# burlachenkok/flpytorch

Measured on AMD Instinct MI355X. Metric: gradient-codec encode+reduce GB/s (device-resident), [N,D] fp32; % HBM peak, higher is better.
Workload: dtype f32; 1 GPU; C3 topk:1% N=1024/GPU D=10000000; codec=topk:1%, clients_per_gpu=1024, clients_total=1024, D=10000000, K=100000, rows_alloc=contiguous, parallelism=client-shard dp1

## Files before the change

flpytorch_amd/csrc/select.hip:

```cpp
#include <stdlib.h>

#include <atomic>
#include <map>
#include <mutex>
#include <vector>

#include "chunks.hpp"
#include "randk_tree.hpp"

namespace flc {

constexpr uint32_t ALL = 0xFFFFFFFFu;
constexpr uint32_t F_OVERFLOW = 1u, F_SHORT = 2u, F_TIES = 4u, F_EXACT = 8u;
constexpr uint32_t F_RESIDENT = 16u;
constexpr uint32_t F_REPAIR = 32u;
constexpr int SMAX = 16384;
constexpr int HBINS = 2048;
constexpr uint32_t TIECAP = HBINS;
constexpr int CS_SH = 64;
constexpr int64_t CS_FEW = 16;
constexpr int CS_ST = 8;
constexpr int CS_LCAP = 2048;
constexpr int RS_U = 16;
#ifndef FLC_RS_NG
// ... 73 lines not shown
    uint32_t* krem;
    uint32_t* tieprefix;
    uint32_t* tiecut;
    uint32_t* hist;
    uint32_t* worklist;
    uint32_t* nwork;
    uint32_t* cursor;
    uint32_t* cstate;
    uint64_t* clist;
    uint32_t* carrive;
    uint32_t* shcnt;
    uint32_t* zm;
    float* part;
    int64_t cap;
    uint32_t tie_hi;
};

__device__ __host__ inline uint32_t tie_pref(uint32_t ix, uint32_t hi) { return hi ? ix : ~ix; }
__device__ __host__ inline uint32_t tie_all(uint32_t hi) { return hi ? 0u : 0xFFFFFFFFu; }


__device__ inline void lds_bar() {
    asm volatile("s_waitcnt lgkmcnt(0)" ::: "memory");
    __builtin_amdgcn_s_barrier();
    asm volatile("" ::: "memory");
}
template <bool RAW>
__device__ inline void blk_bar() {
    if (RAW) lds_bar();
    else __syncthreads();
}
// ... 201 lines not shown
        for (int i = threadIdx.x; i < HBINS; i += NT) ws.hist[row * HBINS + i] = 0;
}

#ifndef FLC_CS_NT
#define FLC_CS_NT 1
#endif
__device__ inline float4 cs_ld(const float4* p) {
#if FLC_CS_NT
    typedef float v4f __attribute__((ext_vector_type(4)));
    const v4f v = __builtin_nontemporal_load(reinterpret_cast<const v4f*>(p));
    return make_float4(v.x, v.y, v.z, v.w);
#else
    return *p;
#endif
}
template <int NT>
__device__ void cand_select_row(int64_t row, int64_t K, SelWs ws, uint32_t* h, uint32_t* scratch) {
    {
        if (ws.flags[row]) return;
        const uint32_t cnt = ws.rowcnt[(row) * RCS];
        if (cnt < (uint32_t)K) {
            if (threadIdx.x == 0) ws.flags[row] |= F_SHORT;
            return;
        }
        const uint32_t T = ws.thr[row];
        const uint32_t span = ws.prefix[row] - T;
        int s = 0;
        while (s < 21 && (((uint64_t)span * 4u) >> s) >= (uint64_t)HBINS) ++s;
        const float* vals = ws.ent_val + row * ws.cap;
        const float4* v4 = reinterpret_cast<const float4*>(vals);
        const uint32_t n4 = cnt >> 2;
        uint32_t prefix = 0, krem = (uint32_t)K, last = 0;
// ... 36 lines not shown
        }
        __syncthreads();
        const uint32_t thr = T + prefix;
        bool ties = !fail && last > krem;
        if (ties && last > TIECAP) { fail = true; ties = false; }
        if (ties) {
            uint32_t* tix = h;
            if (threadIdx.x == 0) scratch[0] = 0;
            __syncthreads();
            const uint32_t* idxs = ws.ent_idx + row * ws.cap;
            for (uint32_t i = threadIdx.x; i < n4; i += NT) {
                const float4 q = v4[i];
                const float qv[4] = {q.x, q.y, q.z, q.w};
#pragma unroll
                for (int u = 0; u < 4; ++u)
                    if (mag_key(qv[u]) == thr) tix[atomicAdd(&scratch[0], 1u)] = idxs[i * 4 + u];
            }
            for (uint32_t i = n4 * 4 + threadIdx.x; i < cnt; i += NT) {
                if (mag_key(vals[i]) == thr) tix[atomicAdd(&scratch[0], 1u)] = idxs[i];
            }
            __syncthreads();
            const uint32_t m = scratch[0];
            for (uint32_t a = threadIdx.x; a < m; a += NT) {
                const uint32_t ia = tix[a];
                uint32_t rank = 0;
                for (uint32_t b = 0; b < m; ++b) rank += tie_pref(tix[b], ws.tie_hi) > tie_pref(ia, ws.tie_hi) ? 1u : 0u;
                if (rank == krem - 1) ws.tiecut[row] = ia;
            }
        }
        if (threadIdx.x == 0) {
            if (fail) {
                ws.flags[row] |= F_SHORT;
            } else {
                ws.thr[row] = thr;
                ws.krem[row] = krem;
                if (ties) ws.flags[row] |= F_TIES;
            }
// ... 351 lines not shown
#define FLC_TK_STPOL 0
#endif
#ifndef FLC_TK_COPY4
#define FLC_TK_COPY4 1
#endif
#ifndef FLC_TK_PROBE
#define FLC_TK_PROBE 0
#endif

template <int POL = FLC_TK_STPOL>
__device__ inline void tk_copy_out(const uint32_t* si, const uint32_t* sv, const SelWs& ws, int64_t n, int64_t row,
                                   uint32_t pos, uint32_t tot, bool fits, int lane, int64_t wslot) {
    int64_t at = row * ws.cap + pos;
    if (FLC_TK_PROBE == 4) at = (wslot % max((n * ws.cap) >> 10, (int64_t)1)) << 10;
    const uint32_t nrec = (fits && FLC_TK_PROBE != 2) ? tot * 4u : 0u;
    const auto di = __builtin_amdgcn_make_buffer_rsrc(ws.ent_idx + at, (short)0, (int)nrec, 0x00020000);
    const auto dv = __builtin_amdgcn_make_buffer_rsrc(ws.ent_val + at, (short)0, (int)nrec, 0x00020000);
    typedef unsigned int u4v __attribute__((ext_vector_type(4)));
    const uint32_t nq = min(tot, (uint32_t)GCAP) >> 2;
#pragma unroll
    for (int k = 0; k < GCAP / 256; ++k) {
        const uint32_t q = (uint32_t)(k * 64 + lane);
        const uint4 a = reinterpret_cast<const uint4*>(si)[q];
        const uint4 b = reinterpret_cast<const uint4*>(sv)[q];
        const uint32_t off = q < nq ? q * 16u : 0x7FFFFFF0u;
        __builtin_amdgcn_raw_buffer_store_b128(__builtin_bit_cast(u4v, a), di, off, 0, POL);
        __builtin_amdgcn_raw_buffer_store_b128(__builtin_bit_cast(u4v, b), dv, off, 0, POL);
    }
    const uint32_t e = nq * 4u + (uint32_t)(lane & 3);
    const uint32_t off = lane < 3 ? e * 4u : 0x7FFFFFF0u;
    __builtin_amdgcn_raw_buffer_store_b32(si[e], di, off, 0, POL);
    __builtin_amdgcn_raw_buffer_store_b32(sv[e], dv, off, 0, POL);
}

template <int RING, int FGS, int LONE = 0>
#ifndef FLC_TK_RING
#define FLC_TK_RING 16
#endif
#ifndef FLC_TK_WPE
#define FLC_TK_WPE 1
#endif
__global__ __launch_bounds__(256) __attribute__((amdgpu_waves_per_eu(FLC_TK_WPE))) void k_topk_filter_fast(RowSrc rows, int64_t n, int64_t r0, int64_t rn, int64_t rb, int64_t d, SelWs ws, int shards,
                                                                                                float* __restrict__ zout) {
    static_assert(16 % RING == 0, "ring must divide the 16 loads of a chunk");
    constexpr int SROW = GCAP + 64;
    static_assert((SROW * 4) % 256 == 0, "value block offset in 256-byte units");
    __shared__ __attribute__((aligned(16))) uint32_t st[2][4][2 * SROW];
// ... 144 lines not shown
#endif
#ifndef FLC_TK_WG_STPOL
#define FLC_TK_WG_STPOL 17
#endif
#ifndef FLC_TK_WG_WPE
#define FLC_TK_WG_WPE 4
#endif
__device__ inline uint32_t lds_addr(const void* p) {
    return (uint32_t)(size_t)(const __attribute__((address_space(3))) void*)p;
}
__device__ inline uint32_t lds_peek(uint32_t addr) {
    uint32_t v;
    asm volatile("ds_read_b32 %0, %1\n\ts_waitcnt lgkmcnt(0)" : "=&v"(v) : "v"(addr) : "memory");
    return __builtin_amdgcn_readfirstlane(v);
}
template <int RING, int NL>
__global__ __launch_bounds__((NL + 1) * 64) __attribute__((amdgpu_waves_per_eu(FLC_TK_WG_WPE))) void k_topk_filter_fast_wg(RowSrc rows, int64_t n, int64_t r0, int64_t rn, int64_t rb, int64_t d,
                                                                        SelWs ws) {
    static_assert(16 % RING == 0, "ring must divide the 16 loads of a chunk");
    constexpr int FGS = 4;
    constexpr int SROW = GCAP + 64;
    __shared__ __attribute__((aligned(16))) uint32_t st[2][NL][2 * SROW];
    __shared__ __attribute__((aligned(16))) uint32_t hs[2][NL][4];
    __shared__ uint32_t fr[2];
    const int lane = threadIdx.x & 63;
    const int wv = __builtin_amdgcn_readfirstlane(threadIdx.x >> 6);
    if (threadIdx.x < 2 * NL * 4) (&hs[0][0][0])[threadIdx.x] = 0;
    if (threadIdx.x < 2) fr[threadIdx.x] = 0;
    __syncthreads();
    const int64_t C = nchunks(d);
    const int64_t G = (C + FGS * NL - 1) / (FGS * NL);
// ... 47 lines not shown
                for (int w = 0; w < NL; ++w)
                    if ((lane >> 2) == w) {
                        off = pre[w];
                        gf = tot[w] <= GCAP;
#pragma unroll
                        for (int u = 0; u < FGS; ++u) {
                            const uint32_t x = (uint32_t)(cc[w] >> (16 * u)) & 0xFFFFu;
                            off += u < (lane & 3) ? x : 0u;
                            cu = u == (lane & 3) ? x : cu;
                        }
                    }
                ws.tab[(c0 + lane) * n + row] = make_uint2(base + off, fits && gf ? cu : 0u);
            }
            if (!(fits && allfit) && lane == 0) atomicOr(&ws.flags[row], F_OVERFLOW);
#pragma unroll
            for (int w = 0; w < NL; ++w)
                tk_copy_out<FLC_TK_WG_STPOL>(st[b][w], st[b][w] + SROW, ws, n, row, base + pre[w], tot[w], fits && tot[w] <= GCAP, lane,
                            (int64_t)blockIdx.x * NL + w);
            asm volatile("s_waitcnt lgkmcnt(0)\n\tds_write_b32 %0, %1" ::"v"(lds_addr(&fr[b])), "v"(k + 1) : "memory");
        }
        return;
    }
    float4 ring[RING];
    int64_t row, c;
    item_at(it, row, c);
    c += wv * FGS;
    auto rs = chunk_rsrc(rows.row_s(row), c * CHUNK, d);
#pragma unroll
    for (int L = 0; L < RING - 1; ++L) {
        ring[L] = load_q(rs, lane, L);
        __builtin_amdgcn_sched_barrier(0);
    }
    for (uint32_t k = 0; it < items; ++k) {
// ... 156 lines not shown
    }
    if (lane == 63) wsum[wv] = inc;
    __syncthreads();
    uint32_t before = 0, tot = 0;
#pragma unroll
    for (int k = 0; k < NT / 64; ++k) {
        const uint32_t x = wsum[k];
        before += k < wv ? x : 0u;
        tot += x;
    }
    __syncthreads();
    total = tot;
    return before + inc - v;
}

template <bool VEC, int NT = EX_NT>
__device__ void exact_row(RowSrc rows, int64_t n, int64_t row, int64_t d, int64_t K, SelWs ws, uint32_t* h,
                          uint32_t* scratch, uint32_t* wsum) {
    const int t = threadIdx.x;
    const int64_t C = nchunks(d);
    {
        const float* r = rows.row(row);
        uint32_t prefix = 0, krem = (uint32_t)K, ties_tot = 0;
        for (int p = 0; p < 3; ++p) {
            for (int i = t; i < HBINS; i += NT) h[i] = 0;
            __syncthreads();
            auto add = [&](uint32_t k) { if (key_in_prefix(k, p, prefix)) atomicAdd(&h[key_bin(k, p)], 1u); };
            int64_t j = 0;
            if (VEC) {
                const float4* r4 = reinterpret_cast<const float4*>(r);
                const int64_t g4 = d / 4;
// ... 54 lines not shown
            }
            uint32_t etot;
            uint32_t erank = tie_run + ex_scan<NT>(ne, wsum, etot);
            uint32_t na = 0;
            bool adm[4];
#pragma unroll
            for (int q = 0; q < 4; ++q) {
                adm[q] = gt[q] || (eq[q] && erank >= tie_from && erank < tie_to);
                erank += eq[q] ? 1u : 0u;
                na += adm[q] ? 1u : 0u;
            }
            uint32_t atot;
            uint32_t pos = base + ex_scan<NT>(na, wsum, atot);
#pragma unroll
            for (int q = 0; q < 4; ++q)
                if (adm[q]) { oi[pos] = (uint32_t)(j0 + q); ov[pos] = v[q]; ++pos; }
            base += atot;
            tie_run += etot;
            if (sb == SUBS - 1 && t == 0) ws.tab[c * n + row] = make_uint2(cbase, base - cbase);
        }
        if (t == 0) {
            ws.thr[row] = thr;
            ws.krem[row] = krem;
            ws.rowcnt[row * RCS] = base;
            ws.flags[row] = F_EXACT | (ws.flags[row] & (F_OVERFLOW | F_SHORT));
        }
        __syncthreads();
    }
}

template <bool VEC>
__global__ __launch_bounds__(EX_NT) void k_topk_exact_rows(RowSrc rows, int64_t n, int64_t r0, int64_t rn, int64_t d, int64_t K, SelWs ws) {
    __shared__ uint32_t h[HBINS];
    __shared__ uint32_t scratch[260];
    __shared__ uint32_t wsum[EX_NT / 64];
    for (int64_t row = r0 + blockIdx.x; row < r0 + rn; row += gridDim.x) {
        if (!(ws.flags[row] & (F_OVERFLOW | F_SHORT))) continue;
        exact_row<VEC>(rows, n, row, d, K, ws, h, scratch, wsum);
    }
}

template <int NT, bool VEC>
__global__ __launch_bounds__(NT) void k_cand_select_x(RowSrc rows, int64_t n, int64_t r0, int64_t rn, int64_t d, int64_t K,
                                                      SelWs ws) {
    __shared__ uint32_t h[HBINS];
    __shared__ uint32_t scratch[260];
    __shared__ uint32_t wsum[NT / 64];
    __shared__ uint32_t failed;
    for (int64_t row = r0 + blockIdx.x; row < r0 + rn; row += gridDim.x) {
        cand_select_row<NT>(row, K, ws, h, scratch);
        __syncthreads();
        if (threadIdx.x == 0) failed = __atomic_load_n(&ws.flags[row], __ATOMIC_RELAXED) & (F_OVERFLOW | F_SHORT);
        __syncthreads();
        if (failed) exact_row<VEC, NT>(rows, n, row, d, K, ws, h, scratch, wsum);
        __syncthreads();
    }
}

__global__ __launch_bounds__(256) void k_tie_count(RowSrc rows, int64_t n, int64_t d, SelWs ws) {
    const int64_t C = nchunks(d);
    const int lane = threadIdx.x & 63, wv = threadIdx.x >> 6;
    const int64_t nrows = *ws.nwork;
    const int64_t bpr = (C + 3) / 4;
    for (int64_t it = blockIdx.x; it < nrows * bpr; it += gridDim.x) {
        const int64_t row = ws.worklist[it / bpr];
        const int64_t c = (it % bpr) * 4 + wv;
        if (c >= C) continue;
        uint32_t cnt = 0;
        if (ws.flags[row] & F_TIES) {
// ... 264 lines not shown
    m.te = make_uint2(0, 0);
    m.thr = 0; m.cut = 0u; m.mode = 0; m.w = 1.f;
    if (r < (rend < 0 ? n : rend)) {
        m.te = ws.tab[c * n + r];
        m.thr = ws.thr[r];
        const uint32_t f = ws.flags[r];
        m.mode = (f & F_EXACT) ? 2u : ((f & F_TIES) ? 1u : 0u);
        if (m.mode == 1u) m.cut = tie_pref(ws.tiecut[r], ws.tie_hi);
        if (m.mode == 2u) m.thr = 0u;
        if (w) m.w = w[r];
    }
    return m;
}


template <int TS>
__device__ void resolve_neg_zero(float* tl, uint32_t* rm, const SelWs& ws, int64_t c, int64_t n, uint32_t cbase,
                                 int64_t len, const float* w, int lane) {
    constexpr int NW = TS / 32;
    constexpr int WL = (NW + 63) / 64;
    bool any = false;
    for (int k = 0; k < TS / 64; ++k) {
        const int64_t i = (int64_t)k * 64 + lane;
        const uint64_t b = __ballot(i < len && __float_as_uint(tl[i]) == 0x80000000u);
        if (lane == 0) { rm[2 * k] = (uint32_t)b; rm[2 * k + 1] = (uint32_t)(b >> 32); }
        any |= b != 0ull;
    }
    if (!any) return;
    uint32_t z0[WL], zc[WL];
#pragma unroll
    for (int j = 0; j < WL; ++j) {
        const int k = lane + 64 * j;
        z0[j] = k < NW ? rm[k] : 0u;
        zc[j] = z0[j];
    }
    for (int64_t r = 0; r < n; ++r) {
        if (w && (__float_as_uint(w[r]) >> 31)) continue;
#pragma unroll
        for (int j = 0; j < WL; ++j) if (lane + 64 * j < NW) rm[lane + 64 * j] = 0u;
        const RowMeta m = load_meta(ws, c, n, r, w);
        const uint32_t mode = m.mode, T = m.thr, cut = m.cut;
        for (uint32_t e = (uint32_t)lane; e < m.te.y; e += 64) {
            const uint32_t ix = ws.ent_idx[r * ws.cap + m.te.x + e];
            const uint32_t key = mag_key(ws.ent_val[r * ws.cap + m.te.x + e]);
            const uint32_t loc = ix - cbase;
            if (loc < (uint32_t)TS && (mode == 2u || key > T || (key == T && tie_pref(ix, ws.tie_hi) >= cut)))
                atomicOr(&rm[loc >> 5], 1u << (loc & 31));
        }
        bool left = false;
#pragma unroll
        for (int j = 0; j < WL; ++j) {
            if (lane + 64 * j < NW) zc[j] &= rm[lane + 64 * j];
            left |= zc[j] != 0u;
        }
        if (__ballot(left) == 0ull) break;
    }
#pragma unroll
    for (int j = 0; j < WL; ++j) {
        uint32_t dead = z0[j] & ~zc[j];
        while (dead) {
            const int b = __builtin_ctz(dead);
            dead &= dead - 1u;
            tl[(lane + 64 * j) * 32 + b] = 0.f;
        }
    }
}

template <int TS>
__device__ void resolve_neg_zero_g(float* tl, uint32_t* rm, const SelWs& ws, int64_t c, int64_t n, uint32_t cbase,
                                   int64_t len, const float* w, int lane) {
    constexpr int NW = TS / 32;
    constexpr int WL = (NW + 63) / 64;
    uint32_t z0[WL], zc[WL];
#pragma unroll
    for (int j = 0; j < WL; ++j) z0[j] = 0u;
    bool any = false;
#pragma unroll 4
    for (int k = 0; k < TS / 64; ++k) {
        const int64_t i = (int64_t)k * 64 + lane;
        const uint64_t b = __ballot(i < len && __float_as_uint(tl[i]) == 0x80000000u);
        const int w0 = 2 * k, w1 = 2 * k + 1;
#pragma unroll
        for (int j = 0; j < WL; ++j) {
// ... 1 lines not shown
            if (lane == (w1 & 63) && (w1 >> 6) == j) z0[j] = (uint32_t)(b >> 32);
        }
        any |= b != 0ull;
    }
    if (!any) return;
#pragma unroll
    for (int j = 0; j < WL; ++j) zc[j] = z0[j];
    for (int64_t r = 0; r < n; ++r) {
        if (w && (__float_as_uint(w[r]) >> 31)) continue;
#pragma unroll
        for (int j = 0; j < WL; ++j) if (lane + 64 * j < NW) rm[lane + 64 * j] = 0u;
        __threadfence_block();
        const RowMeta m = load_meta(ws, c, n, r, w);
        const uint32_t mode = m.mode, T = m.thr, cut = m.cut;
        for (uint32_t e = (uint32_t)lane; e < m.te.y; e += 64) {
            const uint32_t ix = ws.ent_idx[r * ws.cap + m.te.x + e];
            const uint32_t key = mag_key(ws.ent_val[r * ws.cap + m.te.x + e]);
            const uint32_t loc = ix - cbase;
            if (loc < (uint32_t)TS && (mode == 2u || key > T || (key == T && tie_pref(ix, ws.tie_hi) >= cut)))
                atomicOr(&rm[loc >> 5], 1u << (loc & 31));
        }
        __threadfence_block();
        bool left = false;
#pragma unroll
        for (int j = 0; j < WL; ++j) {
            if (lane + 64 * j < NW) zc[j] &= atomicOr(&rm[lane + 64 * j], 0u);
            left |= zc[j] != 0u;
        }
        if (__ballot(left) == 0ull) break;
    }
#pragma unroll
    for (int j = 0; j < WL; ++j) {
        uint32_t dead = z0[j] & ~zc[j];
        while (dead) {
            const int b = __builtin_ctz(dead);
            dead &= dead - 1u;
            tl[(lane + 64 * j) * 32 + b] = 0.f;
        }
    }
}

template <bool ASSIGN, int TS, bool W, int WPB, int AP = AP>
__device__ __forceinline__ void chunk_accum_body(int64_t n, int64_t d, SelWs ws, const float* __restrict__ w, float wt,
                                                 float* __restrict__ out, int64_t r0, int64_t rend, int first, int last,
                                                 float (*tile)[TS], uint32_t (*zmask)[WPB == 1 ? 1 : TS / 32]) {
    if (rend < 0) rend = n;
    constexpr int PARTS = CHUNK / TS;
    const int lane = threadIdx.x & 63;
    const int wv = WPB == 1 ? 0 : __builtin_amdgcn_readfirstlane(threadIdx.x >> 6);
    const int64_t C = nchunks(d);
    float* tl = tile[wv];
    const int64_t nb = (rend - r0 + 63) / 64;
    for (int64_t t = (int64_t)blockIdx.x * WPB + wv; t < C * PARTS; t += (int64_t)gridDim.x * WPB) {
        const int64_t c = t / PARTS;
        const uint32_t cbase = (uint32_t)(c * CHUNK + (t % PARTS) * TS);
        if (FLC_TILE_V4 && !ASSIGN && !first && (int64_t)cbase + TS <= d) {
            const float4* p4 = reinterpret_cast<const float4*>(ws.part + cbase);
// ... 3 lines not shown
#pragma unroll
                for (int k = 0; k < 8; ++k) v[k] = k0 + k < TS / 256 ? p4[(k0 + k) * 64 + lane] : make_float4(0.f, 0.f, 0.f, 0.f);
#pragma unroll
                for (int k = 0; k < 8; ++k)
                    if (k0 + k < TS / 256) reinterpret_cast<float4*>(tl)[(k0 + k) * 64 + lane] = v[k];
            }
        } else {
            for (int i = lane; i < TS; i += 64)
                tl[i] = ASSIGN ? 0.f : (first || (int64_t)cbase + i >= d ? -0.f : ws.part[cbase + i]);
        }
        RowMeta cur = load_meta(ws, c, n, r0 + lane, w, rend), nxt;
        uint32_t ri[AP][2];
        float rv[AP][2];
        auto fetch = [&](const RowMeta& m, int q, int64_t row, int slot) {
            const uint32_t off = __builtin_amdgcn_readlane(m.te.x, q), cnt = __builtin_amdgcn_readlane(m.te.y, q);
            const auto di = list_rsrc(ws.ent_idx + row * ws.cap + off, cnt);
            const auto dv = list_rsrc(ws.ent_val + row * ws.cap + off, cnt);
#pragma unroll
            for (int h = 0; h < 2; ++h) {
                const uint32_t e = (uint32_t)lane + 64u * h;
                const uint32_t x = __builtin_amdgcn_raw_buffer_load_b32(di, lane * 4, h * 256, 0);
                ri[slot][h] = e < cnt ? x : 0xFFFFFFFFu;
                rv[slot][h] = __uint_as_float(__builtin_amdgcn_raw_buffer_load_b32(dv, lane * 4, h * 256, 0));
            }
        };
        const uint32_t txm = ws.tie_hi ? 0u : 0xFFFFFFFFu;
        auto fold = [&](uint32_t ix, float vv, uint32_t T, uint32_t cut, uint32_t mode, float wi) {
            (void)mode;
            const uint32_t loc = ix - cbase;
            const uint64_t a = ((uint64_t)mag_key(vv) << 32) | (uint64_t)(ix ^ txm);
            const uint64_t b = ((uint64_t)T << 32) | (uint64_t)cut;
            if (FLC_CA_PROBE == 1) {
                if (loc < (uint32_t)TS && a >= b && vv == 1.2345f) tl[0] = vv;
                return;
            }
            if (loc < (uint32_t)TS && a >= b) {
// ... 23 lines not shown
                for (int q = 0; q < 64; ++q) {
                    const int slot = q % AP;
                    const uint32_t T = __shfl(cur.thr, q, WAVE), cut = __shfl(cur.cut, q, WAVE);
                    const uint32_t mode = __shfl(cur.mode, q, WAVE), cnt = __shfl(cur.te.y, q, WAVE);
                    const uint32_t off = __shfl(cur.te.x, q, WAVE);
                    const float wi = W ? __shfl(cur.w, q, WAVE) : 1.f;
                    uint32_t i_0 = 0, i_1 = 0;
                    float v_0 = 0.f, v_1 = 0.f;
#pragma unroll
                    for (int z = 0; z < AP; ++z)
                        if (z == slot) { i_0 = ri[z][0]; i_1 = ri[z][1]; v_0 = rv[z][0]; v_1 = rv[z][1]; }
                    fold(i_0, v_0, T, cut, mode, wi);
                    fold(i_1, v_1, T, cut, mode, wi);
                    const int64_t row = i0 + q;
                    for (uint32_t e = 128u + lane; e < cnt; e += 64)
                        fold(ws.ent_idx[row * ws.cap + off + e], ws.ent_val[row * ws.cap + off + e], T, cut, mode, wi);
                    const RowMeta& m = (q + AP < 64) ? cur : nxt;
                    const int qq = (q + AP) & 63;
                    const uint32_t offn = __shfl(m.te.x, qq, WAVE), cntn = __shfl(m.te.y, qq, WAVE);
                    const int64_t rown = i0 + q + AP;
                    uint32_t xi[2];
                    float xv[2];
#pragma unroll
                    for (int h = 0; h < 2; ++h) {
                        const uint32_t e = (uint32_t)lane + 64u * h;
                        xi[h] = e < cntn ? ws.ent_idx[rown * ws.cap + offn + e] : 0xFFFFFFFFu;
                        xv[h] = e < cntn ? ws.ent_val[rown * ws.cap + offn + e] : 0.f;
                    }
#pragma unroll
                    for (int z = 0; z < AP; ++z)
                        if (z == slot) { ri[z][0] = xi[0]; ri[z][1] = xi[1]; rv[z][0] = xv[0]; rv[z][1] = xv[1]; }
                }
            }
            cur = nxt;
        }
        const int64_t len = min((int64_t)TS, d - (int64_t)cbase);
        if (!last) {
            for (int64_t i = lane; i < len; i += 64) ws.part[cbase + i] = tl[i];
            continue;
        }
        if (!ASSIGN) {
            if (WPB == 1) resolve_neg_zero_g<TS>(tl, ws.zm + t * (TS / 32), ws, c, n, cbase, len, w, lane);
            else resolve_neg_zero<TS>(tl, zmask[wv], ws, c, n, cbase, len, w, lane);
        }
        for (int64_t i = lane; i < len; i += 64) out[cbase + i] = ASSIGN ? tl[i] : tl[i] / wt;
    }
}

template <bool ASSIGN, int TS = CHUNK, bool W = true>
__global__ __launch_bounds__(256) void k_chunk_accum(int64_t n, int64_t d, SelWs ws, const float* __restrict__ w, float wt,
                                                     float* __restrict__ out, int64_t r0 = 0, int64_t rend = -1,
                                                     int first = 1, int last = 1) {
    __shared__ __attribute__((aligned(16))) float tile[4][TS];
    __shared__ uint32_t zmask[4][TS / 32];
    chunk_accum_body<ASSIGN, TS, W, 4>(n, d, ws, w, wt, out, r0, rend, first, last, tile, zmask);
}

template <bool W>
__global__ __launch_bounds__(64) void k_chunk_accum1(
        int64_t n, int64_t d, SelWs ws, const float* __restrict__ w, float wt, float* __restrict__ out, int64_t r0,
        int64_t rend, int first, int last) {
    extern __shared__ __attribute__((aligned(16))) float dyn_tile[];
    chunk_accum_body<false, CHUNK, W, 1, FLC_CA_AP1>(n, d, ws, w, wt, out, r0, rend, first, last,
                                         reinterpret_cast<float (*)[CHUNK]>(dyn_tile), nullptr);
}

struct RkdWs {
    uint32_t* cnt;
    uint64_t* ckey;
};

constexpr int RKC_NT = 1024;
constexpr int64_t RKC_BINS = 32768;

__global__ __launch_bounds__(256) void k_randk_ckeys(int64_t n, uint64_t seed, int64_t client0, uint64_t* __restrict__ ckey) {
    const int64_t row = (int64_t)blockIdx.x * 256 + threadIdx.x;
    if (row < n) ckey[row] = client_key(seed, client0 + row);
}
// ... 1192 lines not shown

static int64_t host_chunks(int64_t d) { return (d + CHUNK - 1) / CHUNK; }

int64_t sel_capacity(int codec, int64_t d, int64_t K) {
    if (codec == FLC_RANDK) return std::max<int64_t>(K, 1);
    int64_t cap = 2 * K + 2 * CHUNK;
    cap = std::min<int64_t>(std::max<int64_t>(cap, 1), std::max<int64_t>(d, 1));
    return (cap + 3) & ~int64_t(3);
}

static SelWs carve_sel(void* base, int codec, int64_t n, int64_t d, int64_t K, size_t* bytes) {
    Carver cv(base);
    const int64_t C = std::max<int64_t>(host_chunks(d), 1), nn = std::max<int64_t>(n, 1);
    SelWs s;
    s.tie_hi = 0;
    s.cap = sel_capacity(codec, d, K);
    s.tab = cv.take<uint2>((size_t)C * nn);
    s.ent_idx = cv.take<uint32_t>((size_t)nn * s.cap);
    s.ent_val = cv.take<float>((size_t)nn * s.cap);
    s.rowcnt = cv.take<uint32_t>((size_t)nn * RCS);
    s.flags = cv.take<uint32_t>(nn);
    s.thr = cv.take<uint32_t>(nn);
    s.prefix = cv.take<uint32_t>(nn);
    s.krem = cv.take<uint32_t>(nn);
    s.worklist = cv.take<uint32_t>(nn);
    s.nwork = cv.take<uint32_t>(4);
    s.zm = cv.take<uint32_t>((size_t)C * (CHUNK / 32));
    s.part = codec == FLC_TOPK ? cv.take<float>((size_t)C * CHUNK) : nullptr;
    if (codec == FLC_TOPK) {
        s.tieprefix = cv.take<uint32_t>((size_t)C * nn);
// ... 88 lines not shown
    return cu[dev];
}
static int lone_path() {
    static const int v = [] { const char* e = tuning_env("FLC_LONE_PATH"); return e ? atoi(e) : FLC_LONE_PATH; }();
    return v;
}

static int filter_group() {
    static const int g = [] {
        const char* e = tuning_env("FLC_FILTER_GS");
        return (e && atoi(e) == 2) ? 2 : 4;
    }();
    return g;
}

template <int FGS>
static void launch_filter(RowSrc rows, int64_t n, int64_t r0, int64_t rn, int64_t d, SelWs ws, hipStream_t st,
                          int shards, float* zout = nullptr) {
    const int64_t waves = rn * ((nchunks(d) + FGS - 1) / FGS);
    const int gw = (int)std::max<int64_t>(1, std::min<int64_t>((waves + 3) / 4, 32768));
    static const int64_t rb = [] {
        const char* e = tuning_env("FLC_TK_RB");
        return e ? std::max<int64_t>(1, atoll(e)) : (int64_t)64;
    }();
    ProfScope _pv(FGS == 4 ? "k_topk_filter_g4" : "k_topk_filter_g2", st);
    if constexpr (FGS == 4 && FLC_TK_WG != 0 && FLC_TK_PROBE != 1 && FLC_TK_PROBE != 3) {
        static const bool wg = [] { const char* e = tuning_env("FLC_FILTER_WG"); return !(e && atoi(e) == 0); }();
        if (wg && shards == 1 && !zout) {
            constexpr int NL = FLC_TK_WG_NL;
            const int64_t items = rn * ((nchunks(d) + 4 * NL - 1) / (4 * NL));
            const int gi = (int)std::max<int64_t>(1, std::min<int64_t>(items, 32768));
            static const int64_t rbw = [] {
                const char* e = tuning_env("FLC_TK_RB");
                return e ? std::max<int64_t>(1, atoll(e)) : (int64_t)16;
            }();
            hipLaunchKernelGGL((k_topk_filter_fast_wg<FLC_TK_WG_RING, NL>), dim3(gi), dim3((NL + 1) * 64), 0, st, rows, n, r0,
                               rn, std::min(rbw, std::max<int64_t>(rn, 1)), d, ws);
            return;
        }
    }
    if (zout)
        hipLaunchKernelGGL((k_topk_filter_fast<FLC_TK_RING, FGS, 1>), dim3(gw), dim3(256), 0, st, rows, n, r0, rn,
                           std::min(rb, std::max<int64_t>(rn, 1)), d, ws, shards, zout);
    else
        hipLaunchKernelGGL((k_topk_filter_fast<FLC_TK_RING, FGS>), dim3(gw), dim3(256), 0, st, rows, n, r0, rn,
                           std::min(rb, std::max<int64_t>(rn, 1)), d, ws, shards, (float*)nullptr);
}

#ifndef FLC_TK_SPLIT_SAMPLE
#define FLC_TK_SPLIT_SAMPLE 1
#endif
#ifndef FLC_TK_LASTPCT
// ... 102 lines not shown
    FLC_CHECK_LAUNCH("k_randk_tab");
    {
        ProfScope _ps("k_randk_gen", st);
        const int64_t gx = std::max<int64_t>(1, std::min<int64_t>((C + 4 * RKG_CPW - 1) / (4 * RKG_CPW), 4096));
        hipLaunchKernelGGL(k_randk_gen, dim3((unsigned)gx, (unsigned)std::min<int64_t>(n, 65535)), dim3(256), 0, st, rows,
                           n, d, rw.ckey, prm->randk_scale, sw);
        FLC_CHECK_LAUNCH("k_randk_gen");
    }
    return launch_chunk_accum(n, d, sw, false, w, wt, out, st);
}

static int launch_group_fold(int64_t n, int64_t d, SelWs ws, const float* w, float wt, float* out, int64_t r0, int64_t r1,
                             bool first, bool last, bool exposed, hipStream_t st) {
    const int64_t C = host_chunks(d);
    ProfScope _ps("k_chunk_accum", st);
    if (!exposed) {
        const int ab = grid_stride_blocks(C, 16384);
        if (w) hipLaunchKernelGGL((k_chunk_accum1<true>), dim3(ab), dim3(64), CHUNK * sizeof(float), st, n, d, ws, w, wt, out, r0, r1,
                                  first ? 1 : 0, last ? 1 : 0);
        else hipLaunchKernelGGL((k_chunk_accum1<false>), dim3(ab), dim3(64), CHUNK * sizeof(float), st, n, d, ws, w, wt, out, r0, r1,
                                first ? 1 : 0, last ? 1 : 0);
    } else {
        constexpr int LTS = FLC_TK_LAST_TS;
        const int ab = grid_stride_blocks((C * (CHUNK / LTS) + 3) / 4, 4096);
        if (w) hipLaunchKernelGGL((k_chunk_accum<false, LTS, true>), dim3(ab), dim3(256), 0, st, n, d, ws, w, wt, out, r0, r1,
                                  first ? 1 : 0, last ? 1 : 0);
        else hipLaunchKernelGGL((k_chunk_accum<false, LTS, false>), dim3(ab), dim3(256), 0, st, n, d, ws, w, wt, out, r0, r1,
                                first ? 1 : 0, last ? 1 : 0);
    }
    FLC_CHECK_LAUNCH("k_chunk_accum(group)");
    return FLC_OK;
}

static int launch_chunk_accum(int64_t n, int64_t d, SelWs ws, bool assign, const float* w, float wt, float* out,
                              hipStream_t st) {
    const int64_t C = host_chunks(d);
    { ProfScope _ps("k_chunk_accum", st);
    int parts = accum_parts();
    if (parts == 0) parts = C >= 1024 ? 1 : (C >= 256 ? 2 : 4);
    auto go = [&](auto ts, int ab) {
        constexpr int TS = decltype(ts)::value;
        if (assign) hipLaunchKernelGGL((k_chunk_accum<true, TS>), dim3(ab), dim3(256), 0, st, n, d, ws, w, wt, out);
        else if (w) hipLaunchKernelGGL((k_chunk_accum<false, TS, true>), dim3(ab), dim3(256), 0, st, n, d, ws, w, wt, out);
        else hipLaunchKernelGGL((k_chunk_accum<false, TS, false>), dim3(ab), dim3(256), 0, st, n, d, ws, w, wt, out);
// ... 96 lines not shown
                FLC_CHECK_LAUNCH("k_lone_resident");
                rc.xcum += (uint32_t)Gu;
                if (FLC_RS_EVREC) FLC_CHECK_HIP(hipEventRecord(rc.done, st));
                rc.last = st;
                return FLC_OK;
            }
        }
        const bool dense_k = K * 16 > d;
        lone_assign = assign && n == 1 && few && !dense_k && !assign_fold();

        if (dense_k) FLC_CHECK_HIP(hipMemsetAsync(ws.hist, 0, (size_t)n * HBINS * sizeof(uint32_t), st));
        const int64_t bpr = (C + 3) / 4;
        if (!dense_k) {
            const int TG = few ? 1 : tk_tail_groups(prm, n);
            gfold = FLC_TK_GFOLD && !few && !assign && !dense_k;
            hipStream_t sside = st;
            TkCtx* cx = nullptr;
            std::unique_lock<std::mutex> lk;
            if (TG > 1) {
                int dev = 0;
                FLC_CHECK_HIP(hipGetDevice(&dev));
                lk = std::unique_lock<std::mutex>(g_tk_mu);
                cx = &g_tk_ctx[dev];
                if (!cx->side) {
                    int lo = 0, hi = 0;
                    FLC_CHECK_HIP(hipDeviceGetStreamPriorityRange(&lo, &hi));
                    FLC_CHECK_HIP(hipStreamCreateWithPriority(&cx->side, hipStreamNonBlocking, hi));
                }
                while ((int)cx->ev.size() < TG + 3) {
                    hipEvent_t e;
// ... 14 lines not shown
                FLC_CHECK_HIP(hipEventRecord(cx->ev[TG + 1], st));
                FLC_CHECK_HIP(hipStreamWaitEvent(sside, cx->ev[TG + 1], 0));
            }
            sample(0, rs1, st);
            FLC_CHECK_LAUNCH("k_topk_sample");
            if (split) {
                sample(rs1, n, sside);
                FLC_CHECK_LAUNCH("k_topk_sample (side)");
                FLC_CHECK_HIP(hipEventRecord(cx->ev[TG + 2], sside));
            }
            for (int g = 0; g < TG; ++g) {
                const int64_t r0 = group_row(n, TG, g, FLC_TK_LASTPCT), rn = group_row(n, TG, g + 1, FLC_TK_LASTPCT) - r0;
                if (split && g == 1) FLC_CHECK_HIP(hipStreamWaitEvent(st, cx->ev[TG + 2], 0));
                { ProfScope _ps("k_topk_filter", st);
                float* zout = lone_assign ? out : nullptr;
                if (filter_group() == 2 || n * d < ((int64_t)64 << 20)) launch_filter<2>(rows, n, r0, rn, d, ws, st, few ? CS_SH : 1, zout);
                else launch_filter<4>(rows, n, r0, rn, d, ws, st, few ? CS_SH : 1, zout); }
                FLC_CHECK_LAUNCH("k_topk_filter");
                if (TG > 1) {
                    FLC_CHECK_HIP(hipEventRecord(cx->ev[g], st));
                    FLC_CHECK_HIP(hipStreamWaitEvent(sside, cx->ev[g], 0));
                }
                { ProfScope _ps("k_cand_select", sside);
                if (few) {
                    const int np = (FLC_CS_LIST && d <= FLC_CS_TWO_MAXD) ? 2 : 3;
                    for (int p = 0; p < np; ++p)
                        hipLaunchKernelGGL(k_cs_pass, dim3((unsigned)CS_SH, (unsigned)n), dim3(CS_NT), 0, st, K, ws,
                                           p == np - 1 ? 1 : 0);
                } else if (gfold) {
                    const bool big = rn < 128 || g == TG - 1;
                    const int nt = big ? 1024 : FLC_TK_SIDE_NT;
                    const dim3 grid((unsigned)(big ? rn : grid_stride_blocks(rn, 8192)));
                    if (big) {
                        if (vec) hipLaunchKernelGGL((k_cand_select_x<1024, true>), grid, dim3(nt), 0, sside, rows, n, r0, rn, d, K, ws);
                        else hipLaunchKernelGGL((k_cand_select_x<1024, false>), grid, dim3(nt), 0, sside, rows, n, r0, rn, d, K, ws);
                    } else if (FLC_TK_SIDE_NT == 256) {
                        if (vec) hipLaunchKernelGGL((k_cand_select_x<256, true>), grid, dim3(nt), 0, sside, rows, n, r0, rn, d, K, ws);
                        else hipLaunchKernelGGL((k_cand_select_x<256, false>), grid, dim3(nt), 0, sside, rows, n, r0, rn, d, K, ws);
                    } else {
                        if (vec) hipLaunchKernelGGL((k_cand_select_x<512, true>), grid, dim3(nt), 0, sside, rows, n, r0, rn, d, K, ws);
                        else hipLaunchKernelGGL((k_cand_select_x<512, false>), grid, dim3(nt), 0, sside, rows, n, r0, rn, d, K, ws);
                    }
                } else if (rn < 128 || (TG > 1 && g == TG - 1))
                    hipLaunchKernelGGL(k_cand_select<1024>, dim3((unsigned)rn), dim3(1024), 0, sside, r0, rn, K, ws);
                else if (FLC_TK_SIDE_NT == 256)
                    hipLaunchKernelGGL(k_cand_select<256>, dim3(grid_stride_blocks(rn, 8192)), dim3(256), 0, sside, r0, rn, K, ws);
                else hipLaunchKernelGGL(k_cand_select<512>, dim3(grid_stride_blocks(rn, 8192)), dim3(512), 0, sside, r0, rn, K, ws); }
                FLC_CHECK_LAUNCH("k_cand_select");
                if (gfold) {
                    const bool lastg = g == TG - 1;
                    if (int rc = launch_group_fold(n, d, ws, w, wt, out, r0, r0 + rn, g == 0, lastg, lastg || TG == 1, sside))
                        return rc;
                }
            }
            if (!lone_assign && !gfold) {
                ProfScope _ps("k_topk_exact_rows", sside);
                const int eb = grid_stride_blocks(n, FLC_TK_EXACT_WG);
// ... 157 lines not shown
```

Before: 5282 GB/s.

## Store candidate indices as 16-bit chunk-local offsets to halve index traffic

Candidate indices written by the top-k filter are stored as 16-bit offsets within their chunk instead of full 32-bit global indices. The chunk base is rebuilt from the per-chunk table in the accumulate, candidate-select tie handling and neg-zero resolution paths. This cuts the bytes written and read for the index stream. In exchange it adds a per-tie scan over all chunks to recover global indices, needs odd-alignment handling for 16-bit buffer stores, and applies only when the group-fold, filter-g4 and workgroup-filter paths are all active.

After: 5359 GB/s, median of 6. 1.01x the previous value.

```diff
diff --git a/flpytorch_amd/csrc/select.hip b/flpytorch_amd/csrc/select.hip
--- a/flpytorch_amd/csrc/select.hip
+++ b/flpytorch_amd/csrc/select.hip
@@ -111,7 +111,12 @@
     float* part;
     int64_t cap;
     uint32_t tie_hi;
+    uint32_t idx16;
 };
+
+__device__ inline uint16_t* idx16_row(const SelWs& ws, int64_t row) {
+    return reinterpret_cast<uint16_t*>(ws.ent_idx + row * ws.cap);
+}
 
 __device__ __host__ inline uint32_t tie_pref(uint32_t ix, uint32_t hi) { return hi ? ix : ~ix; }
 __device__ __host__ inline uint32_t tie_all(uint32_t hi) { return hi ? 0u : 0xFFFFFFFFu; }
@@ -343,8 +348,9 @@
     return *p;
 #endif
 }
-template <int NT>
-__device__ void cand_select_row(int64_t row, int64_t K, SelWs ws, uint32_t* h, uint32_t* scratch) {
+template <int NT, bool I16 = false>
+__device__ void cand_select_row(int64_t row, int64_t K, SelWs ws, uint32_t* h, uint32_t* scratch, int64_t n = 0,
+                                int64_t C = 0) {
     {
         if (ws.flags[row]) return;
         const uint32_t cnt = ws.rowcnt[(row) * RCS];
@@ -411,13 +417,28 @@
                 const float qv[4] = {q.x, q.y, q.z, q.w};
 #pragma unroll
                 for (int u = 0; u < 4; ++u)
-                    if (mag_key(qv[u]) == thr) tix[atomicAdd(&scratch[0], 1u)] = idxs[i * 4 + u];
+                    if (mag_key(qv[u]) == thr) tix[atomicAdd(&scratch[0], 1u)] = I16 ? i * 4 + u : idxs[i * 4 + u];
             }
             for (uint32_t i = n4 * 4 + threadIdx.x; i < cnt; i += NT) {
-                if (mag_key(vals[i]) == thr) tix[atomicAdd(&scratch[0], 1u)] = idxs[i];
+                if (mag_key(vals[i]) == thr) tix[atomicAdd(&scratch[0], 1u)] = I16 ? i : idxs[i];
             }
             __syncthreads();
             const uint32_t m = scratch[0];
+            if constexpr (I16) {
+                uint32_t* gix = ws.hist + row * HBINS;
+                const uint16_t* l16 = idx16_row(ws, row);
+                for (int64_t c = threadIdx.x; c < C; c += NT) {
+                    const uint2 te = ws.tab[c * n + row];
+                    if (te.y == 0u) continue;
+                    for (uint32_t a = 0; a < m; ++a) {
+                        const uint32_t pp = tix[a];
+                        if (pp - te.x < te.y) gix[a] = (uint32_t)(c << CHUNK_SHIFT) + l16[pp];
+                    }
+                }
+                __syncthreads();
+                for (uint32_t a = threadIdx.x; a < m; a += NT) tix[a] = gix[a];
+                __syncthreads();
+            }
             for (uint32_t a = threadIdx.x; a < m; a += NT) {
                 const uint32_t ia = tix[a];
                 uint32_t rank = 0;
@@ -799,7 +820,7 @@
     int64_t at = row * ws.cap + pos;
     if (FLC_TK_PROBE == 4) at = (wslot % max((n * ws.cap) >> 10, (int64_t)1)) << 10;
     const uint32_t nrec = (fits && FLC_TK_PROBE != 2) ? tot * 4u : 0u;
-    const auto di = __builtin_amdgcn_make_buffer_rsrc(ws.ent_idx + at, (short)0, (int)nrec, 0x00020000);
+    const auto di = __builtin_amdgcn_make_buffer_rsrc(ws.ent_idx + at, (short)0, FLC_TK_PROBE == 5 ? 0 : (int)nrec, 0x00020000);
     const auto dv = __builtin_amdgcn_make_buffer_rsrc(ws.ent_val + at, (short)0, (int)nrec, 0x00020000);
     typedef unsigned int u4v __attribute__((ext_vector_type(4)));
     const uint32_t nq = min(tot, (uint32_t)GCAP) >> 2;
@@ -816,6 +837,53 @@
     const uint32_t off = lane < 3 ? e * 4u : 0x7FFFFFF0u;
     __builtin_amdgcn_raw_buffer_store_b32(si[e], di, off, 0, POL);
     __builtin_amdgcn_raw_buffer_store_b32(sv[e], dv, off, 0, POL);
+}
+
+template <int POL>
+__device__ inline void tk_copy_out16(const uint32_t* si, const uint32_t* sv, const SelWs& ws, int64_t n, int64_t row,
+                                     uint32_t pos, uint32_t tot, bool fits, int lane, int64_t wslot) {
+    static_assert(GCAP == 512, "one 16-B index store per lane covers the group");
+    int64_t at = row * ws.cap + pos;
+    int64_t at16 = 2 * row * ws.cap + pos;
+    if (FLC_TK_PROBE == 4) at16 = at = (wslot % max((n * ws.cap) >> 10, (int64_t)1)) << 10;
+    const uint32_t nrec = (fits && FLC_TK_PROBE != 2) ? tot * 4u : 0u;
+    const uint32_t lead = (uint32_t)at16 & 1u;
+    const uint32_t nrec16 = (fits && FLC_TK_PROBE != 2 && FLC_TK_PROBE != 5) ? (tot + lead) * 2u : 0u;
+    const auto di = __builtin_amdgcn_make_buffer_rsrc(reinterpret_cast<uint16_t*>(ws.ent_idx) + (at16 - lead), (short)0, (int)nrec16, 0x00020000);
+    const auto dv = __builtin_amdgcn_make_buffer_rsrc(ws.ent_val + at, (short)0, (int)nrec, 0x00020000);
+    typedef unsigned int u4v __attribute__((ext_vector_type(4)));
+    const uint32_t tc = min(tot, (uint32_t)GCAP);
+    const uint32_t nq = tc >> 2;
+#pragma unroll
+    for (int k = 0; k < GCAP / 256; ++k) {
+        const uint32_t q = (uint32_t)(k * 64 + lane);
+        const uint4 b = reinterpret_cast<const uint4*>(sv)[q];
+        const uint32_t off = q < nq ? q * 16u : 0x7FFFFFF0u;
+        __builtin_amdgcn_raw_buffer_store_b128(__builtin_bit_cast(u4v, b), dv, off, 0, POL);
+    }
+    {
+        const uint32_t e = nq * 4u + (uint32_t)(lane & 3);
+        const uint32_t off = lane < 3 ? e * 4u : 0x7FFFFFF0u;
+        __builtin_amdgcn_raw_buffer_store_b32(sv[e], dv, off, 0, POL);
+    }
+    const uint32_t ld0 = tc ? lead : 0u;
+    const uint32_t n8 = (tc - ld0) >> 3;
+    {
+        const uint32_t e0 = ld0 + (uint32_t)lane * 8u;
+        uint32_t p[4];
+#pragma unroll
+        for (int j = 0; j < 4; ++j)
+            p[j] = (si[e0 + 2 * j] & (uint32_t)(CHUNK - 1)) | ((si[e0 + 2 * j + 1] & (uint32_t)(CHUNK - 1)) << 16);
+        const u4v a = {p[0], p[1], p[2], p[3]};
+        const uint32_t off = (uint32_t)lane < n8 ? (lead + ld0 + (uint32_t)lane * 8u) * 2u : 0x7FFFFFF0u;
+        __builtin_amdgcn_raw_buffer_store_b128(a, di, off, 0, POL);
+    }
+    {
+        const uint32_t e = lane == 7 ? 0u : ld0 + n8 * 8u + (uint32_t)lane;
+        const bool on = lane == 7 ? ld0 != 0u : (lane < 7 && e < tc);
+        const uint32_t off = on ? (lead + e) * 2u : 0x7FFFFFF0u;
+        __builtin_amdgcn_raw_buffer_store_b16((unsigned short)(si[on ? e : 0u] & (uint32_t)(CHUNK - 1)), di, off, 0, POL);
+    }
 }
 
 template <int RING, int FGS, int LONE = 0>
@@ -990,7 +1058,10 @@
     asm volatile("ds_read_b32 %0, %1\n\ts_waitcnt lgkmcnt(0)" : "=&v"(v) : "v"(addr) : "memory");
     return __builtin_amdgcn_readfirstlane(v);
 }
-template <int RING, int NL>
+#ifndef FLC_TK_IDX16
+#define FLC_TK_IDX16 1
+#endif
+template <int RING, int NL, bool I16 = false>
 __global__ __launch_bounds__((NL + 1) * 64) __attribute__((amdgpu_waves_per_eu(FLC_TK_WG_WPE))) void k_topk_filter_fast_wg(RowSrc rows, int64_t n, int64_t r0, int64_t rn, int64_t rb, int64_t d,
                                                                         SelWs ws) {
     static_assert(16 % RING == 0, "ring must divide the 16 loads of a chunk");
@@ -1068,9 +1139,14 @@
             }
             if (!(fits && allfit) && lane == 0) atomicOr(&ws.flags[row], F_OVERFLOW);
 #pragma unroll
-            for (int w = 0; w < NL; ++w)
-                tk_copy_out<FLC_TK_WG_STPOL>(st[b][w], st[b][w] + SROW, ws, n, row, base + pre[w], tot[w], fits && tot[w] <= GCAP, lane,
-                            (int64_t)blockIdx.x * NL + w);
+            for (int w = 0; w < NL; ++w) {
+                if constexpr (I16)
+                    tk_copy_out16<FLC_TK_WG_STPOL>(st[b][w], st[b][w] + SROW, ws, n, row, base + pre[w], tot[w], fits && tot[w] <= GCAP, lane,
+                                                   (int64_t)blockIdx.x * NL + w);
+                else
+                    tk_copy_out<FLC_TK_WG_STPOL>(st[b][w], st[b][w] + SROW, ws, n, row, base + pre[w], tot[w], fits && tot[w] <= GCAP, lane,
+                                                 (int64_t)blockIdx.x * NL + w);
+            }
             asm volatile("s_waitcnt lgkmcnt(0)\n\tds_write_b32 %0, %1" ::"v"(lds_addr(&fr[b])), "v"(k + 1) : "memory");
         }
         return;
@@ -1257,7 +1333,7 @@
     return before + inc - v;
 }
 
-template <bool VEC, int NT = EX_NT>
+template <bool VEC, int NT = EX_NT, bool I16 = false>
 __device__ void exact_row(RowSrc rows, int64_t n, int64_t row, int64_t d, int64_t K, SelWs ws, uint32_t* h,
                           uint32_t* scratch, uint32_t* wsum) {
     const int t = threadIdx.x;
@@ -1342,7 +1418,12 @@
             uint32_t pos = base + ex_scan<NT>(na, wsum, atot);
 #pragma unroll
             for (int q = 0; q < 4; ++q)
-                if (adm[q]) { oi[pos] = (uint32_t)(j0 + q); ov[pos] = v[q]; ++pos; }
+                if (adm[q]) {
+                    if constexpr (I16) reinterpret_cast<uint16_t*>(oi)[pos] = (uint16_t)((j0 + q) & (CHUNK - 1));
+                    else oi[pos] = (uint32_t)(j0 + q);
+                    ov[pos] = v[q];
+                    ++pos;
+                }
             base += atot;
             tie_run += etot;
             if (sb == SUBS - 1 && t == 0) ws.tab[c * n + row] = make_uint2(cbase, base - cbase);
@@ -1368,7 +1449,7 @@
     }
 }
 
-template <int NT, bool VEC>
+template <int NT, bool VEC, bool I16 = false>
 __global__ __launch_bounds__(NT) void k_cand_select_x(RowSrc rows, int64_t n, int64_t r0, int64_t rn, int64_t d, int64_t K,
                                                       SelWs ws) {
     __shared__ uint32_t h[HBINS];
@@ -1376,11 +1457,11 @@
     __shared__ uint32_t wsum[NT / 64];
     __shared__ uint32_t failed;
     for (int64_t row = r0 + blockIdx.x; row < r0 + rn; row += gridDim.x) {
-        cand_select_row<NT>(row, K, ws, h, scratch);
+        cand_select_row<NT, I16>(row, K, ws, h, scratch, n, nchunks(d));
         __syncthreads();
         if (threadIdx.x == 0) failed = __atomic_load_n(&ws.flags[row], __ATOMIC_RELAXED) & (F_OVERFLOW | F_SHORT);
         __syncthreads();
-        if (failed) exact_row<VEC, NT>(rows, n, row, d, K, ws, h, scratch, wsum);
+        if (failed) exact_row<VEC, NT, I16>(rows, n, row, d, K, ws, h, scratch, wsum);
         __syncthreads();
     }
 }
@@ -1675,7 +1756,7 @@
 }
 
 
-template <int TS>
+template <int TS, bool I16 = false>
 __device__ void resolve_neg_zero(float* tl, uint32_t* rm, const SelWs& ws, int64_t c, int64_t n, uint32_t cbase,
                                  int64_t len, const float* w, int lane) {
     constexpr int NW = TS / 32;
@@ -1702,7 +1783,7 @@
         const RowMeta m = load_meta(ws, c, n, r, w);
         const uint32_t mode = m.mode, T = m.thr, cut = m.cut;
         for (uint32_t e = (uint32_t)lane; e < m.te.y; e += 64) {
-            const uint32_t ix = ws.ent_idx[r * ws.cap + m.te.x + e];
+            const uint32_t ix = I16 ? (uint32_t)(c << CHUNK_SHIFT) + idx16_row(ws, r)[m.te.x + e] : ws.ent_idx[r * ws.cap + m.te.x + e];
             const uint32_t key = mag_key(ws.ent_val[r * ws.cap + m.te.x + e]);
             const uint32_t loc = ix - cbase;
             if (loc < (uint32_t)TS && (mode == 2u || key > T || (key == T && tie_pref(ix, ws.tie_hi) >= cut)))
@@ -1727,7 +1808,7 @@
     }
 }
 
-template <int TS>
+template <int TS, bool I16 = false>
 __device__ void resolve_neg_zero_g(float* tl, uint32_t* rm, const SelWs& ws, int64_t c, int64_t n, uint32_t cbase,
                                    int64_t len, const float* w, int lane) {
     constexpr int NW = TS / 32;
@@ -1759,7 +1840,7 @@
         const RowMeta m = load_meta(ws, c, n, r, w);
         const uint32_t mode = m.mode, T = m.thr, cut = m.cut;
         for (uint32_t e = (uint32_t)lane; e < m.te.y; e += 64) {
-            const uint32_t ix = ws.ent_idx[r * ws.cap + m.te.x + e];
+            const uint32_t ix = I16 ? (uint32_t)(c << CHUNK_SHIFT) + idx16_row(ws, r)[m.te.x + e] : ws.ent_idx[r * ws.cap + m.te.x + e];
             const uint32_t key = mag_key(ws.ent_val[r * ws.cap + m.te.x + e]);
             const uint32_t loc = ix - cbase;
             if (loc < (uint32_t)TS && (mode == 2u || key > T || (key == T && tie_pref(ix, ws.tie_hi) >= cut)))
@@ -1785,7 +1866,7 @@
     }
 }
 
-template <bool ASSIGN, int TS, bool W, int WPB, int AP = AP>
+template <bool ASSIGN, int TS, bool W, int WPB, int AP = AP, bool I16 = false>
 __device__ __forceinline__ void chunk_accum_body(int64_t n, int64_t d, SelWs ws, const float* __restrict__ w, float wt,
                                                  float* __restrict__ out, int64_t r0, int64_t rend, int first, int last,
                                                  float (*tile)[TS], uint32_t (*zmask)[WPB == 1 ? 1 : TS / 32]) {
@@ -1819,12 +1900,15 @@
         float rv[AP][2];
         auto fetch = [&](const RowMeta& m, int q, int64_t row, int slot) {
             const uint32_t off = __builtin_amdgcn_readlane(m.te.x, q), cnt = __builtin_amdgcn_readlane(m.te.y, q);
-            const auto di = list_rsrc(ws.ent_idx + row * ws.cap + off, cnt);
             const auto dv = list_rsrc(ws.ent_val + row * ws.cap + off, cnt);
+            const uint32_t odd = I16 ? off & 1u : 0u;
+            const auto di = I16 ? __builtin_amdgcn_make_buffer_rsrc(idx16_row(ws, row) + (off - odd), (short)0, (int)((cnt + odd) * 2u), 0x00020000)
+                                : list_rsrc(ws.ent_idx + row * ws.cap + off, cnt);
 #pragma unroll
             for (int h = 0; h < 2; ++h) {
                 const uint32_t e = (uint32_t)lane + 64u * h;
-                const uint32_t x = __builtin_amdgcn_raw_buffer_load_b32(di, lane * 4, h * 256, 0);
+                const uint32_t x = I16 ? (uint32_t)(c << CHUNK_SHIFT) + (uint32_t)__builtin_amdgcn_raw_buffer_load_b16(di, (lane + odd) * 2, h * 128, 0)
+                                       : __builtin_amdgcn_raw_buffer_load_b32(di, lane * 4, h * 256, 0);
                 ri[slot][h] = e < cnt ? x : 0xFFFFFFFFu;
                 rv[slot][h] = __uint_as_float(__builtin_amdgcn_raw_buffer_load_b32(dv, lane * 4, h * 256, 0));
             }
@@ -1878,7 +1962,8 @@
                     fold(i_1, v_1, T, cut, mode, wi);
                     const int64_t row = i0 + q;
                     for (uint32_t e = 128u + lane; e < cnt; e += 64)
-                        fold(ws.ent_idx[row * ws.cap + off + e], ws.ent_val[row * ws.cap + off + e], T, cut, mode, wi);
+                        fold(I16 ? (uint32_t)(c << CHUNK_SHIFT) + idx16_row(ws, row)[off + e] : ws.ent_idx[row * ws.cap + off + e],
+                             ws.ent_val[row * ws.cap + off + e], T, cut, mode, wi);
                     const RowMeta& m = (q + AP < 64) ? cur : nxt;
                     const int qq = (q + AP) & 63;
                     const uint32_t offn = __shfl(m.te.x, qq, WAVE), cntn = __shfl(m.te.y, qq, WAVE);
@@ -1888,7 +1973,8 @@
 #pragma unroll
                     for (int h = 0; h < 2; ++h) {
                         const uint32_t e = (uint32_t)lane + 64u * h;
-                        xi[h] = e < cntn ? ws.ent_idx[rown * ws.cap + offn + e] : 0xFFFFFFFFu;
+                        xi[h] = e >= cntn ? 0xFFFFFFFFu
+                              : I16 ? (uint32_t)(c << CHUNK_SHIFT) + idx16_row(ws, rown)[offn + e] : ws.ent_idx[rown * ws.cap + offn + e];
                         xv[h] = e < cntn ? ws.ent_val[rown * ws.cap + offn + e] : 0.f;
                     }
 #pragma unroll
@@ -1904,28 +1990,28 @@
             continue;
         }
         if (!ASSIGN) {
-            if (WPB == 1) resolve_neg_zero_g<TS>(tl, ws.zm + t * (TS / 32), ws, c, n, cbase, len, w, lane);
-            else resolve_neg_zero<TS>(tl, zmask[wv], ws, c, n, cbase, len, w, lane);
+            if (WPB == 1) resolve_neg_zero_g<TS, I16>(tl, ws.zm + t * (TS / 32), ws, c, n, cbase, len, w, lane);
+            else resolve_neg_zero<TS, I16>(tl, zmask[wv], ws, c, n, cbase, len, w, lane);
         }
         for (int64_t i = lane; i < len; i += 64) out[cbase + i] = ASSIGN ? tl[i] : tl[i] / wt;
     }
 }
 
-template <bool ASSIGN, int TS = CHUNK, bool W = true>
+template <bool ASSIGN, int TS = CHUNK, bool W = true, bool I16 = false>
 __global__ __launch_bounds__(256) void k_chunk_accum(int64_t n, int64_t d, SelWs ws, const float* __restrict__ w, float wt,
                                                      float* __restrict__ out, int64_t r0 = 0, int64_t rend = -1,
                                                      int first = 1, int last = 1) {
     __shared__ __attribute__((aligned(16))) float tile[4][TS];
     __shared__ uint32_t zmask[4][TS / 32];
-    chunk_accum_body<ASSIGN, TS, W, 4>(n, d, ws, w, wt, out, r0, rend, first, last, tile, zmask);
-}
-
-template <bool W>
+    chunk_accum_body<ASSIGN, TS, W, 4, AP, I16>(n, d, ws, w, wt, out, r0, rend, first, last, tile, zmask);
+}
+
+template <bool W, bool I16 = false>
 __global__ __launch_bounds__(64) void k_chunk_accum1(
         int64_t n, int64_t d, SelWs ws, const float* __restrict__ w, float wt, float* __restrict__ out, int64_t r0,
         int64_t rend, int first, int last) {
     extern __shared__ __attribute__((aligned(16))) float dyn_tile[];
-    chunk_accum_body<false, CHUNK, W, 1, FLC_CA_AP1>(n, d, ws, w, wt, out, r0, rend, first, last,
+    chunk_accum_body<false, CHUNK, W, 1, FLC_CA_AP1, I16>(n, d, ws, w, wt, out, r0, rend, first, last,
                                          reinterpret_cast<float (*)[CHUNK]>(dyn_tile), nullptr);
 }
 
@@ -3148,6 +3234,7 @@
     const int64_t C = std::max<int64_t>(host_chunks(d), 1), nn = std::max<int64_t>(n, 1);
     SelWs s;
     s.tie_hi = 0;
+    s.idx16 = 0;
     s.cap = sel_capacity(codec, d, K);
     s.tab = cv.take<uint2>((size_t)C * nn);
     s.ent_idx = cv.take<uint32_t>((size_t)nn * s.cap);
@@ -3266,6 +3353,11 @@
     return g;
 }
 
+static bool filter_wg_on() {
+    if (FLC_TK_WG == 0 || FLC_TK_PROBE == 1 || FLC_TK_PROBE == 3) return false;
+    static const bool wg = [] { const char* e = tuning_env("FLC_FILTER_WG"); return !(e && atoi(e) == 0); }();
+    return wg;
+}
 template <int FGS>
 static void launch_filter(RowSrc rows, int64_t n, int64_t r0, int64_t rn, int64_t d, SelWs ws, hipStream_t st,
                           int shards, float* zout = nullptr) {
@@ -3277,8 +3369,7 @@
     }();
     ProfScope _pv(FGS == 4 ? "k_topk_filter_g4" : "k_topk_filter_g2", st);
     if constexpr (FGS == 4 && FLC_TK_WG != 0 && FLC_TK_PROBE != 1 && FLC_TK_PROBE != 3) {
-        static const bool wg = [] { const char* e = tuning_env("FLC_FILTER_WG"); return !(e && atoi(e) == 0); }();
-        if (wg && shards == 1 && !zout) {
+        if (filter_wg_on() && shards == 1 && !zout) {
             constexpr int NL = FLC_TK_WG_NL;
             const int64_t items = rn * ((nchunks(d) + 4 * NL - 1) / (4 * NL));
             const int gi = (int)std::max<int64_t>(1, std::min<int64_t>(items, 32768));
@@ -3286,8 +3377,12 @@
                 const char* e = tuning_env("FLC_TK_RB");
                 return e ? std::max<int64_t>(1, atoll(e)) : (int64_t)16;
             }();
-            hipLaunchKernelGGL((k_topk_filter_fast_wg<FLC_TK_WG_RING, NL>), dim3(gi), dim3((NL + 1) * 64), 0, st, rows, n, r0,
-                               rn, std::min(rbw, std::max<int64_t>(rn, 1)), d, ws);
+            if (ws.idx16)
+                hipLaunchKernelGGL((k_topk_filter_fast_wg<FLC_TK_WG_RING, NL, true>), dim3(gi), dim3((NL + 1) * 64), 0, st, rows, n, r0,
+                                   rn, std::min(rbw, std::max<int64_t>(rn, 1)), d, ws);
+            else
+                hipLaunchKernelGGL((k_topk_filter_fast_wg<FLC_TK_WG_RING, NL>), dim3(gi), dim3((NL + 1) * 64), 0, st, rows, n, r0,
+                                   rn, std::min(rbw, std::max<int64_t>(rn, 1)), d, ws);
             return;
         }
     }
@@ -3420,20 +3515,25 @@
                              bool first, bool last, bool exposed, hipStream_t st) {
     const int64_t C = host_chunks(d);
     ProfScope _ps("k_chunk_accum", st);
-    if (!exposed) {
-        const int ab = grid_stride_blocks(C, 16384);
-        if (w) hipLaunchKernelGGL((k_chunk_accum1<true>), dim3(ab), dim3(64), CHUNK * sizeof(float), st, n, d, ws, w, wt, out, r0, r1,
-                                  first ? 1 : 0, last ? 1 : 0);
-        else hipLaunchKernelGGL((k_chunk_accum1<false>), dim3(ab), dim3(64), CHUNK * sizeof(float), st, n, d, ws, w, wt, out, r0, r1,
-                                first ? 1 : 0, last ? 1 : 0);
-    } else {
-        constexpr int LTS = FLC_TK_LAST_TS;
-        const int ab = grid_stride_blocks((C * (CHUNK / LTS) + 3) / 4, 4096);
-        if (w) hipLaunchKernelGGL((k_chunk_accum<false, LTS, true>), dim3(ab), dim3(256), 0, st, n, d, ws, w, wt, out, r0, r1,
-                                  first ? 1 : 0, last ? 1 : 0);
-        else hipLaunchKernelGGL((k_chunk_accum<false, LTS, false>), dim3(ab), dim3(256), 0, st, n, d, ws, w, wt, out, r0, r1,
-                                first ? 1 : 0, last ? 1 : 0);
-    }
+    auto go = [&](auto i16) {
+        constexpr bool I = decltype(i16)::value;
+        if (!exposed) {
+            const int ab = grid_stride_blocks(C, 16384);
+            if (w) hipLaunchKernelGGL((k_chunk_accum1<true, I>), dim3(ab), dim3(64), CHUNK * sizeof(float), st, n, d, ws, w, wt, out, r0, r1,
+                                      first ? 1 : 0, last ? 1 : 0);
+            else hipLaunchKernelGGL((k_chunk_accum1<false, I>), dim3(ab), dim3(64), CHUNK * sizeof(float), st, n, d, ws, w, wt, out, r0, r1,
+                                    first ? 1 : 0, last ? 1 : 0);
+        } else {
+            constexpr int LTS = FLC_TK_LAST_TS;
+            const int ab = grid_stride_blocks((C * (CHUNK / LTS) + 3) / 4, 4096);
+            if (w) hipLaunchKernelGGL((k_chunk_accum<false, LTS, true, I>), dim3(ab), dim3(256), 0, st, n, d, ws, w, wt, out, r0, r1,
+                                      first ? 1 : 0, last ? 1 : 0);
+            else hipLaunchKernelGGL((k_chunk_accum<false, LTS, false, I>), dim3(ab), dim3(256), 0, st, n, d, ws, w, wt, out, r0, r1,
+                                    first ? 1 : 0, last ? 1 : 0);
+        }
+    };
+    if (ws.idx16) go(std::true_type{});
+    else go(std::false_type{});
     FLC_CHECK_LAUNCH("k_chunk_accum(group)");
     return FLC_OK;
 }
@@ -3560,6 +3660,8 @@
         if (!dense_k) {
             const int TG = few ? 1 : tk_tail_groups(prm, n);
             gfold = FLC_TK_GFOLD && !few && !assign && !dense_k;
+            const bool fg4 = !(filter_group() == 2 || n * d < ((int64_t)64 << 20));
+            ws.idx16 = (FLC_TK_IDX16 && gfold && fg4 && filter_wg_on() && !lone_assign) ? 1u : 0u;
             hipStream_t sside = st;
             TkCtx* cx = nullptr;
             std::unique_lock<std::mutex> lk;
@@ -3604,7 +3706,7 @@
                 if (split && g == 1) FLC_CHECK_HIP(hipStreamWaitEvent(st, cx->ev[TG + 2], 0));
                 { ProfScope _ps("k_topk_filter", st);
                 float* zout = lone_assign ? out : nullptr;
-                if (filter_group() == 2 || n * d < ((int64_t)64 << 20)) launch_filter<2>(rows, n, r0, rn, d, ws, st, few ? CS_SH : 1, zout);
+                if (!fg4) launch_filter<2>(rows, n, r0, rn, d, ws, st, few ? CS_SH : 1, zout);
                 else launch_filter<4>(rows, n, r0, rn, d, ws, st, few ? CS_SH : 1, zout); }
                 FLC_CHECK_LAUNCH("k_topk_filter");
                 if (TG > 1) {
@@ -3621,16 +3723,21 @@
                     const bool big = rn < 128 || g == TG - 1;
                     const int nt = big ? 1024 : FLC_TK_SIDE_NT;
                     const dim3 grid((unsigned)(big ? rn : grid_stride_blocks(rn, 8192)));
-                    if (big) {
-                        if (vec) hipLaunchKernelGGL((k_cand_select_x<1024, true>), grid, dim3(nt), 0, sside, rows, n, r0, rn, d, K, ws);
-                        else hipLaunchKernelGGL((k_cand_select_x<1024, false>), grid, dim3(nt), 0, sside, rows, n, r0, rn, d, K, ws);
-                    } else if (FLC_TK_SIDE_NT == 256) {
-                        if (vec) hipLaunchKernelGGL((k_cand_select_x<256, true>), grid, dim3(nt), 0, sside, rows, n, r0, rn, d, K, ws);
-                        else hipLaunchKernelGGL((k_cand_select_x<256, false>), grid, dim3(nt), 0, sside, rows, n, r0, rn, d, K, ws);
-                    } else {
-                        if (vec) hipLaunchKernelGGL((k_cand_select_x<512, true>), grid, dim3(nt), 0, sside, rows, n, r0, rn, d, K, ws);
-                        else hipLaunchKernelGGL((k_cand_select_x<512, false>), grid, dim3(nt), 0, sside, rows, n, r0, rn, d, K, ws);
-                    }
+                    auto go = [&](auto i16) {
+                        constexpr bool I = decltype(i16)::value;
+                        if (big) {
+                            if (vec) hipLaunchKernelGGL((k_cand_select_x<1024, true, I>), grid, dim3(nt), 0, sside, rows, n, r0, rn, d, K, ws);
+                            else hipLaunchKernelGGL((k_cand_select_x<1024, false, I>), grid, dim3(nt), 0, sside, rows, n, r0, rn, d, K, ws);
+                        } else if (FLC_TK_SIDE_NT == 256) {
+                            if (vec) hipLaunchKernelGGL((k_cand_select_x<256, true, I>), grid, dim3(nt), 0, sside, rows, n, r0, rn, d, K, ws);
+                            else hipLaunchKernelGGL((k_cand_select_x<256, false, I>), grid, dim3(nt), 0, sside, rows, n, r0, rn, d, K, ws);
+                        } else {
+                            if (vec) hipLaunchKernelGGL((k_cand_select_x<512, true, I>), grid, dim3(nt), 0, sside, rows, n, r0, rn, d, K, ws);
+                            else hipLaunchKernelGGL((k_cand_select_x<512, false, I>), grid, dim3(nt), 0, sside, rows, n, r0, rn, d, K, ws);
+                        }
+                    };
+                    if (ws.idx16) go(std::true_type{});
+                    else go(std::false_type{});
                 } else if (rn < 128 || (TG > 1 && g == TG - 1))
                     hipLaunchKernelGGL(k_cand_select<1024>, dim3((unsigned)rn), dim3(1024), 0, sside, r0, rn, K, ws);
                 else if (FLC_TK_SIDE_NT == 256)
```
